# rfonod/geo-trax

Hardware: AMD Instinct MI355X
Metric: 4K frames/sec through detect+stabilize+track (higher is better)
Workload: dtype f32 (split-f16x3 MFMA)

## Files before the change

### geo-trax_amd/csrc/det_kernels.hip

```cpp
#include <hip/hip_runtime.h>

#include <mutex>
#include <hip/hip_fp16.h>

#include <cmath>

#include "det_kernels.hpp"

namespace gtx {

typedef _Float16 half8 __attribute__((ext_vector_type(8)));
typedef _Float16 half4 __attribute__((ext_vector_type(4)));

namespace {
inline double py_round(double v) { return std::nearbyint(v); }
}

Letterbox letterbox_geometry(int src_h, int src_w, int imgsz, bool rect, int stride) {
  Letterbox lb{};
  lb.src_h = src_h;
  lb.src_w = src_w;
  const double r = std::min((double)imgsz / src_h, (double)imgsz / src_w);
  lb.new_w = (int)py_round(src_w * r);
  lb.new_h = (int)py_round(src_h * r);
// ... 749 lines not shown

template <typename T> __device__ __forceinline__ float ldf(const T* p) { return (float)*p; }

__device__ __forceinline__ int find_level(const HeadParams& hp, int a) {
  int l = 0;
#pragma unroll
  for (int i = 1; i < kMaxLevels; ++i)
    if (i < hp.n_levels && a >= hp.lv[i].anchor_begin) l = i;
  return l;
}

template <typename T> __device__ __forceinline__ void load8(const T* p, float (&v)[8]);
template <> __device__ __forceinline__ void load8<_Float16>(const _Float16* p, float (&v)[8]) {
  const half8 h = *reinterpret_cast<const half8*>(p);
#pragma unroll
  for (int i = 0; i < 8; ++i) v[i] = (float)h[i];
}
template <> __device__ __forceinline__ void load8<float>(const float* p, float (&v)[8]) {
  const float4 a = reinterpret_cast<const float4*>(p)[0], b = reinterpret_cast<const float4*>(p)[1];
  v[0] = a.x; v[1] = a.y; v[2] = a.z; v[3] = a.w; v[4] = b.x; v[5] = b.y; v[6] = b.z; v[7] = b.w;
}

template <typename T>
__global__ __launch_bounds__(256) void head_candidates_kernel(const HeadParams hp, const NmsBuffers nb) {
  const int sub = threadIdx.x & 15;
  const int a = blockIdx.x * 16 + (threadIdx.x >> 4);
  const int n = blockIdx.y;
  const bool valid = a < hp.n_anchors;
  const int l = find_level(hp, valid ? a : 0);
  const HeadLevel& L = hp.lv[l];
  const int la = (valid ? a : 0) - L.anchor_begin;
  const T* fc = static_cast<const T*>(L.feat) + ((size_t)n * L.h * L.w + la) * L.cstride + L.cb;
  const int chunks = L.cc >> 3;
  float best = -1.f;
  int best_c = 0;
  for (int c0 = 0; c0 < hp.nc; c0 += 4) {
    float acc[4] = {0.f, 0.f, 0.f, 0.f};
    for (int ch = sub; ch < chunks; ch += 16) {
      float f[8];
      load8<T>(fc + ch * 8, f);
#pragma unroll
      for (int j = 0; j < 4; ++j) {
        if (c0 + j < hp.nc) {
          float w[8];
          load8<float>(L.wc + (size_t)(c0 + j) * L.cc + ch * 8, w);
#pragma unroll
          for (int e = 0; e < 8; ++e) acc[j] = fmaf(f[e], w[e], acc[j]);
// ... 92 lines not shown
}

template <typename T>
__global__ __launch_bounds__(256) void head_raw_kernel(const HeadParams hp, float* __restrict__ out, int logits) {
  const int n = blockIdx.y;
  const int lane = threadIdx.x & 63;
  const int a = (blockIdx.x * blockDim.x + threadIdx.x) >> 6;
  if (a >= hp.n_anchors) return;
  const int l = find_level(hp, a);
  const HeadLevel& L = hp.lv[l];
  const int la = a - L.anchor_begin;
  const T* f = static_cast<const T*>(L.feat) + ((size_t)n * L.h * L.w + la) * L.cstride;
  const float4 b = anchor_box<T>(L, f, la, lane);
  float* o = out + ((size_t)n * hp.n_anchors + a) * (4 + hp.nc);
  if (lane == 0) { o[0] = b.x; o[1] = b.y; o[2] = b.z; o[3] = b.w; }
  const T* fc = f + L.cb;
  for (int c = lane; c < hp.nc; c += 64) {
    float acc = L.bc[c];
    for (int k = 0; k < L.cc; ++k) acc = fmaf(ldf(fc + k), L.wc[c * L.cc + k], acc);
    o[4 + c] = logits ? acc : 1.f / (1.f + expf(-acc));
  }
}

void launch_head_candidates(int dtype, const HeadParams& hp, int n, const NmsBuffers& nb, hipStream_t s) {
  launch_head_gate(dtype, hp, n, nb, s);
  launch_head_boxes(dtype, hp, n, nb, s);
}

void launch_head_gate(int dtype, const HeadParams& hp, int n, const NmsBuffers& nb, hipStream_t s) {
  GTX_HIP(hipMemsetAsync(nb.count, 0, sizeof(int) * n, s));
  if (nb.lvl_count) GTX_HIP(hipMemsetAsync(nb.lvl_count, 0, sizeof(int) * n * kMaxLevels, s));
  dim3 grid(cdiv(hp.n_anchors, 16), n), block(256);
  if (dtype == DT_F16) hipLaunchKernelGGL(head_candidates_kernel<_Float16>, grid, block, 0, s, hp, nb);
  else hipLaunchKernelGGL(head_candidates_kernel<float>, grid, block, 0, s, hp, nb);
  GTX_HIP(hipGetLastError());
}

void launch_head_boxes(int dtype, const HeadParams& hp, int n, const NmsBuffers& nb, hipStream_t s) {
  dim3 grid2(64, n), block(256);
  const size_t lds = (size_t)hp.n_levels * hp.lv[0].cb * 64 * sizeof(float);
  GTX_CHECK(hp.n_levels <= kMaxLevels && hp.lv[0].cb <= 128, "head: %d levels of %d box channels", hp.n_levels, hp.lv[0].cb);
  static std::once_flag once;
  std::call_once(once, [] {
    GTX_HIP(hipFuncSetAttribute(reinterpret_cast<const void*>(head_boxes_kernel<_Float16>), hipFuncAttributeMaxDynamicSharedMemorySize, kMaxLevels * 128 * 64 * 4));
    GTX_HIP(hipFuncSetAttribute(reinterpret_cast<const void*>(head_boxes_kernel<float>), hipFuncAttributeMaxDynamicSharedMemorySize, kMaxLevels * 128 * 64 * 4));
  });
  if (dtype == DT_F16) hipLaunchKernelGGL(head_boxes_kernel<_Float16>, grid2, block, lds, s, hp, nb);
  else hipLaunchKernelGGL(head_boxes_kernel<float>, grid2, block, lds, s, hp, nb);
  GTX_HIP(hipGetLastError());
}

void launch_head_raw(int dtype, const HeadParams& hp, int n, float* out, bool logits, hipStream_t s) {
  dim3 grid(cdiv(hp.n_anchors * 64, 256), n), block(256);
  if (dtype == DT_F16) hipLaunchKernelGGL(head_raw_kernel<_Float16>, grid, block, 0, s, hp, out, logits ? 1 : 0);
  else hipLaunchKernelGGL(head_raw_kernel<float>, grid, block, 0, s, hp, out, logits ? 1 : 0);
  GTX_HIP(hipGetLastError());
}
// ... 163 lines not shown
    if (nb.out_anchor) nb.out_anchor[(size_t)n * nb.max_det + slot] = nb.s_anchor[(size_t)n * nb.nms_cap + i];
  }
}


__device__ __forceinline__ bool iou_gt(const float4& a, float area_a, const float4& b, float thr) {
  const float iw = fminf(a.z, b.z) - fmaxf(a.x, b.x);
  const float ih = fminf(a.w, b.w) - fmaxf(a.y, b.y);
  if (!(iw > 0.f && ih > 0.f)) return false;
  const float area_b = (b.z - b.x) * (b.w - b.y);
  const float inter = iw * ih;
  return inter / (area_a + area_b - inter) > thr;
}

__global__ __launch_bounds__(1024) void nms_small_kernel(const NmsBuffers nb, float thr, float cls_offset, float gain, float padx,
                                                         float pady, float fw, float fh) {
  __shared__ unsigned long long s_key[kSmallNms];
  __shared__ float4 s_box[kSmallNms];
  __shared__ float4 s_kbox[kSmallKeep];
  __shared__ int s_nkeep, s_done;
  const int n = blockIdx.x;
  const int tid = threadIdx.x, lane = tid & 63;
  const int wave = __builtin_amdgcn_readfirstlane(tid >> 6), nwaves = blockDim.x >> 6;
  const int cnt = min(nb.count[n], nb.cap);
  if (cnt > kSmallNms || nb.max_det > kSmallKeep) {
    if (tid == 0) nb.out_n[n] = 0;
    return;
  }
  if (tid == 0) { nb.sorted_n[n] = 0; s_nkeep = 0; s_done = 0; }
  const size_t base = (size_t)n * nb.cap;
  int P = 64;
  while (P < cnt) P <<= 1;
  for (int i = tid; i < P; i += blockDim.x) {
    unsigned long long k = 0ull;
    if (i < cnt) {
      const unsigned sb = __float_as_uint(nb.cand_score[base + i]);
      k = ((unsigned long long)sb << 32) | ((unsigned long long)(0x7FFFFu - (unsigned)nb.cand_anchor[base + i]) << 12) | (unsigned)i;
    }
    s_key[i] = k;
  }
  __syncthreads();
  for (int k = 2; k <= P; k <<= 1)
    for (int j = k >> 1; j > 0; j >>= 1) {
      for (int t = tid; t < P / 2; t += blockDim.x) {
        const int lo = ((t / j) * 2 * j) + (t % j), hi = lo + j;
        const bool desc = ((lo & k) == 0);
// ... 143 lines not shown
```

### geo-trax_amd/csrc/det_kernels.hpp

```cpp
#pragma once
#include <vector>

#include "common.hpp"
#include "conv_igemm.hpp"

namespace gtx {

struct Letterbox {
  int src_h, src_w;
  int net_h, net_w;
  int new_h, new_w;
  int top, left;
  double gain;
};
Letterbox letterbox_geometry(int src_h, int src_w, int imgsz, bool rect, int stride);

void launch_preprocess(int dtype, const uint8_t* frames, int n, const Letterbox& lb, void* img,
                       uint8_t* gray, int gh, int gw, hipStream_t s);

void launch_stem(int dtype, const void* img, int n, int h, int w, const float* w27, const float* bias,
                 const void* wpk_f16, int c0, void* out, int ho, int wo, hipStream_t s, float acc_scale = 1.f);
std::vector<uint16_t> pack_stem_weights_f16(const float* w27, int c0);
std::vector<uint16_t> pack_stem_weights_split(const float* w27, int c0, float* acc_scale);

// ... 24 lines not shown
};

struct NmsBuffers {
  int cap;
  int* count;
  float* cand_score;
  int* cand_anchor;
  int* cand_cls;
  float* cand_box;
  int nms_cap;
  int* sorted_n;
  float* s_box;
  float* s_score;
  int* s_cls;
  int* s_anchor;
  unsigned long long* mask;
  int max_det;
  int* out_n;
  float* out_rows;
  int* out_anchor;
  int* lvl_count;
  int* lvl_list;
  int lvl_cap;
};

struct FeatLevels {
  const void* feat[kMaxLevels];
  int h[kMaxLevels], w[kMaxLevels], cstride[kMaxLevels], coff[kMaxLevels], c[kMaxLevels];
  int anchor_begin[kMaxLevels];
  int n_levels;
  int dim;
};
void launch_obj_feats(int dtype, const FeatLevels& fl, int n, const NmsBuffers& nb, float* out, hipStream_t s);

void launch_head_candidates(int dtype, const HeadParams& hp, int n, const NmsBuffers& nb, hipStream_t s);
void launch_head_gate(int dtype, const HeadParams& hp, int n, const NmsBuffers& nb, hipStream_t s);
void launch_head_boxes(int dtype, const HeadParams& hp, int n, const NmsBuffers& nb, hipStream_t s);

struct SparseBoxLevel {
  const void* in;
  int H, W, cstride, coff, cin;
  const void* w1; const float* b1; float sc1;
  const void* w2; const float* b2; float sc2;
  int anchor_begin;
  const float* wb; const float* bb; float stride;
};
struct SparseBox {
  SparseBoxLevel lv[kMaxLevels];
  int n_levels;
  int cap;
  int* sat_flag;
};
void launch_head_sparse_box(const SparseBox& sb, int n, const NmsBuffers& nb, hipStream_t s);
void launch_head_raw(int dtype, const HeadParams& hp, int n, float* out, bool logits, hipStream_t s);
void launch_nms(const NmsBuffers& nb, int n, float iou_thr, bool agnostic, int max_nms,
                const Letterbox& lb, hipStream_t s, int which = 0);
bool nms_small_covers(int candidates, int max_det);

}
// ... 1 lines not shown
```

### geo-trax_amd/csrc/detector.cpp

```cpp
#include "detector.hpp"
#include "split_format.hpp"

#include <algorithm>
#include <array>
#include <cmath>
#include <deque>
#include <functional>
#include <mutex>

namespace gtx {

Detector::Detector(gtx_ctx* ctx, const gtx_det_config& cfg) : ctx_(ctx), cfg_(cfg) {
  GTX_CHECK(cfg.imgsz > 0 && cfg.imgsz % 32 == 0, "imgsz must be a positive multiple of 32 (got %d)", cfg.imgsz);
  GTX_CHECK(cfg.max_det > 0 && cfg.nc > 0 && cfg.nc <= 128, "max_det must be positive and nc in [1, 128] (got %d, %d)", cfg.max_det, cfg.nc);
  GTX_CHECK(cfg.frame_h > 0 && cfg.frame_w > 0, "frame size must be given");
  if (cfg_.max_batch < 1) cfg_.max_batch = 1;
  dtype_ = cfg.half ? DT_F16 : DT_F32;
  conv_dtype_ = (!cfg.half && cfg.fp32_split) ? DT_F32S : dtype_;
  es_ = dtype_size(dtype_);
  lb_ = letterbox_geometry(cfg.frame_h, cfg.frame_w, cfg.imgsz, cfg.rect != 0, 32);
  GTX_CHECK(lb_.net_h % 32 == 0 && lb_.net_w % 32 == 0, "network input %dx%d is not stride aligned", lb_.net_h, lb_.net_w);
  GTX_HIP(hipSetDevice(ctx->device));
  for (auto& e : ev_) GTX_HIP(hipEventCreateWithFlags(&e, wait_event_flags(true)));
  for (auto& e : ev_up_) GTX_HIP(hipEventCreate(&e));
}

Detector::~Detector() {
  if (h_out_n_) (void)hipHostFree(h_out_n_);
  if (h_sat_) (void)hipHostFree(h_sat_);
  if (h_out_rows_) (void)hipHostFree(h_out_rows_);
  if (h_feats_) (void)hipHostFree(h_feats_);
  if (h_count_) (void)hipHostFree(h_count_);
  for (auto& e : ev_)
    if (e) (void)hipEventDestroy(e);
  for (auto& e : ev_up_)
    if (e) (void)hipEventDestroy(e);
  for (auto& e : trace_ev_)
    if (e) (void)hipEventDestroy(e);
  if (graph_exec_) (void)hipGraphExecDestroy(graph_exec_);
}

void Detector::set_tensor(const std::string& name, const float* data, int ndim, const int64_t* shape) {
  GTX_CHECK(!finalized_, "set_tensor after finalize");
  HostTensor t;
  size_t n = 1;
  for (int i = 0; i < ndim; ++i) {
    t.shape.push_back(shape[i]);
    n *= (size_t)shape[i];
  }
  t.data.assign(data, data + n);
  tensors_[name] = std::move(t);
}

const HostTensor& Detector::tensor(const std::string& name) const {
  auto it = tensors_.find(name);
// ... 156 lines not shown
  int n = 0;
  while (has(pfx + ".m." + std::to_string(n) + ".cv1.conv.weight")) ++n;
  View cat = new_view(x.h, x.w, (2 + n) * c);
  View first = cat.slice(0, 2 * c);
  conv(pfx + ".cv1.conv", x, 1, true, &first, nullptr, up_src);
  for (int k = 0; k < n; ++k) {
    View tmp = new_view(x.h, x.w, c);
    const std::string m = pfx + ".m." + std::to_string(k);
    View src = cat.slice((1 + k) * c, c);
    View dst = cat.slice((2 + k) * c, c);
    conv(m + ".cv1.conv", src, 1, true, &tmp, nullptr);
    conv(m + ".cv2.conv", tmp, 1, true, &dst, shortcut ? &src : nullptr);
  }
  View out = conv(pfx + ".cv2.conv", cat, 1, true, out_slice, nullptr);
  layer_views_[pfx] = out;
  return out;
}

void Detector::build_graph() {
  const int H = lb_.net_h, W = lb_.net_w;
  img_ = new_view(H, W, 4);
  if (conv_dtype_ == DT_F32S) {
    sat_dev_ = (int*)alloc(sizeof(int));
    GTX_HIP(hipHostMalloc((void**)&h_sat_, sizeof(int)));
    *h_sat_ = 0;
  }

  const HostTensor& w0 = tensor("model.0.conv.weight");
  GTX_CHECK(w0.shape.size() == 4 && w0.shape[1] == 3 && w0.shape[2] == 3, "model.0 must be a 3x3 conv on 3 channels");
  const int c0 = (int)w0.shape[0];
  View a0 = new_view(H / 2, W / 2, c0);
  {
    std::vector<float> w27((size_t)27 * c0);
    for (int o = 0; o < c0; ++o)
      for (int i = 0; i < 3; ++i)
        for (int y = 0; y < 3; ++y)
          for (int x = 0; x < 3; ++x)
            w27[(size_t)((y * 3 + x) * 3 + i) * c0 + o] = w0.data[(((size_t)o * 3 + i) * 3 + y) * 3 + x];
    float* dw = (float*)alloc(w27.size() * sizeof(float));
    GTX_HIP(hipMemcpy(dw, w27.data(), w27.size() * sizeof(float), hipMemcpyHostToDevice));
    std::vector<float> b(c0, 0.f);
    if (has("model.0.conv.bias")) b = tensor("model.0.conv.bias").data;
    float* db = (float*)alloc((size_t)(c0 + 31) / 32 * 32 * sizeof(float));
    GTX_HIP(hipMemcpy(db, b.data(), c0 * sizeof(float), hipMemcpyHostToDevice));
    Op op;
    op.kind = Op::STEM;
    op.name = "model.0.conv";
    op.family = dtype_ == DT_F16 ? "stem_mfma_kernel" : (conv_dtype_ == DT_F32S ? "stem_split_kernel" : "stem_kernel");
// ... 533 lines not shown
    pad_skip_rows_ = 0;
    for (Op& op : ops_)
      for (int i = 0; i < kMaxGroup; ++i) op.ty_first[i] = op.ty_count[i] = 0;
    return;
  }
  pad_skip_on_ = true;
}

void Detector::finalize() {
  GTX_CHECK(!finalized_, "finalize called twice");
  GTX_HIP(hipSetDevice(ctx_->device));
  build_graph();
  fuse_front();
  fuse_stem();
  release_hidden_layers();
  const int N = cfg_.max_batch;
  gray_h_ = cfg_.frame_h / 2;
  gray_w_ = cfg_.frame_w / 2;
  gray_.alloc((size_t)kGrayRing * N * gray_h_ * gray_w_);
  nms_ = NmsBuffers{};
  nms_.cap = head_.n_anchors;
  nms_.nms_cap = 30016;
  nms_.max_det = cfg_.max_det;
  nms_.count = (int*)alloc(sizeof(int) * N);
  nms_.cand_score = (float*)alloc(sizeof(float) * N * nms_.cap);
  nms_.cand_anchor = (int*)alloc(sizeof(int) * N * nms_.cap);
  nms_.cand_cls = (int*)alloc(sizeof(int) * N * nms_.cap);
  nms_.cand_box = (float*)alloc(sizeof(float) * 4 * N * nms_.cap);
  nms_.sorted_n = (int*)alloc(sizeof(int) * N);
  nms_.s_box = (float*)alloc(sizeof(float) * 4 * N * nms_.nms_cap);
  nms_.s_score = (float*)alloc(sizeof(float) * N * nms_.nms_cap);
  nms_.s_cls = (int*)alloc(sizeof(int) * N * nms_.nms_cap);
  nms_.mask = (unsigned long long*)alloc(sizeof(unsigned long long) * N * (size_t)nms_.nms_cap * (nms_.nms_cap / 64));
  nms_.out_n = (int*)alloc(sizeof(int) * N);
  nms_.out_rows = (float*)alloc(sizeof(float) * 6 * N * cfg_.max_det);
  nms_.s_anchor = nms_.out_anchor = nullptr;
  if (cfg_.obj_feats) {
    nms_.s_anchor = (int*)alloc(sizeof(int) * N * nms_.nms_cap);
    nms_.out_anchor = (int*)alloc(sizeof(int) * N * cfg_.max_det);
    d_feats_ = (float*)alloc(sizeof(float) * N * cfg_.max_det * feat_levels_.dim);
    GTX_HIP(hipHostMalloc((void**)&h_feats_, sizeof(float) * N * cfg_.max_det * feat_levels_.dim));
  }
  if (sparse_on_) {
    sparse_.cap = kSparseCap;
    sparse_.sat_flag = sat_dev_;
    nms_.lvl_cap = kSparseCap;
    nms_.lvl_count = (int*)alloc(sizeof(int) * N * kMaxLevels);
    nms_.lvl_list = (int*)alloc(sizeof(int) * N * kMaxLevels * kSparseCap);
  }
  GTX_HIP(hipHostMalloc((void**)&h_count_, sizeof(int) * N));
  GTX_HIP(hipHostMalloc((void**)&h_out_n_, sizeof(int) * N));
  GTX_HIP(hipHostMalloc((void**)&h_out_rows_, sizeof(float) * 6 * N * cfg_.max_det));
  if (conv_dtype_ != DT_F32S) tensors_.clear();
  if (env_flag("GTX_PAD_SKIP", true)) {
    plan_pad_skip();
    prime_pad_skip();
  }
  set_batch(1);
  GTX_HIP(hipStreamSynchronize(ctx_->stream));
  finalized_ = true;
}

void Detector::run_op(const Op& op, int nb, hipStream_t s) {
  switch (op.kind) {
    case Op::CONV:
      conv_launch(op.grp, op.cfg, s);
      break;
    case Op::STEM:
      launch_stem(dtype_ == DT_F32 ? conv_dtype_ : dtype_, op.in.ptr, nb, op.in.h, op.in.w, op.w27, op.bias, op.wpk, op.out.c, op.out.ptr, op.out.h,
                  op.out.w, s, op.stem_scale);
      break;
    case Op::POOL: launch_sppf_pool(conv_dtype_ == DT_F32S ? DT_F32S : dtype_, op.out.ptr, nb, op.in.h, op.in.w, op.in.c, s); break;
    case Op::UPSAMPLE:
      launch_upsample2x(dtype_, op.in.ptr, nb, op.in.h, op.in.w, op.in.c, op.in.cstride, op.in.coff, op.out.ptr,
                        op.out.cstride, op.out.coff, s);
// ... 51 lines not shown
  for (size_t i = 0; i < ops_.size() && i < trace_n_.size(); ++i) {
    if (trace_n_[i] == 0) continue;
    auto it = idx.find(ops_[i].family);
    size_t k;
    if (it == idx.end()) {
      k = names.size();
      idx[ops_[i].family] = k;
      names.push_back(ops_[i].family);
      launches.push_back(0); ms.push_back(0.f); flops.push_back(0.0); bytes.push_back(0.0);
    } else {
      k = it->second;
    }
    launches[k] += trace_n_[i];
    ms[k] += (float)trace_ms_[i];
    flops[k] += trace_flops_[i];
    bytes[k] += trace_bytes_[i];
  }
  trace_ms_.assign(ops_.size(), 0.0);
  trace_n_.assign(ops_.size(), 0);
  trace_flops_.assign(ops_.size(), 0.0);
  trace_bytes_.assign(ops_.size(), 0.0);
}

void Detector::run_post(int nb, hipStream_t s) {
  if (sparse_on_) {
    launch_head_gate(dtype_, head_, nb, nms_, s);
    launch_head_sparse_box(sparse_, nb, nms_, s);
    dense_head_valid_ = false;
  } else {
    launch_head_candidates(dtype_, head_, nb, nms_, s);
  }
  GTX_HIP(hipMemcpyAsync(h_count_, nms_.count, sizeof(int) * nb, hipMemcpyDeviceToHost, s));
  launch_nms(nms_, nb, cfg_.iou, cfg_.agnostic_nms != 0, 30000, lb_, s, 1);
  GTX_HIP(hipMemcpyAsync(h_out_n_, nms_.out_n, sizeof(int) * nb, hipMemcpyDeviceToHost, s));
  GTX_HIP(hipMemcpyAsync(h_out_rows_, nms_.out_rows, sizeof(float) * 6 * nb * cfg_.max_det, hipMemcpyDeviceToHost, s));
  if (sat_dev_) GTX_HIP(hipMemcpyAsync(h_sat_, sat_dev_, sizeof(int), hipMemcpyDeviceToHost, s));
  if (cfg_.obj_feats) {
    launch_obj_feats(conv_dtype_, feat_levels_, nb, nms_, d_feats_, s);
    GTX_HIP(hipMemcpyAsync(h_feats_, d_feats_, sizeof(float) * nb * cfg_.max_det * feat_levels_.dim, hipMemcpyDeviceToHost, s));
  }
}

void Detector::run_dense_box(hipStream_t s) {
  if (!sparse_on_ || dense_head_valid_) return;
  GTX_CHECK(cur_nb_ > 0, "no forward pass has run yet");
  for (Op o : dense_box_ops_) {
    for (int i = 0; i < o.grp.count; ++i) o.grp.p[i].N = cur_nb_;
    conv_group_finalize(o.grp, o.cfg);
    run_op(o, cur_nb_, s);
  }
  dense_head_valid_ = true;
}

void Detector::features(int b, float* out, int cap, int* n, int* dim) const {
  if (exact_) return exact_->features(b, out, cap, n, dim);
  GTX_CHECK(cfg_.obj_feats && h_feats_, "features: the detector was created without gtx_det_config.obj_feats");
  GTX_CHECK(b >= 0 && b < cfg_.max_batch, "features: image %d of %d", b, cfg_.max_batch);
  const int cnt = std::min(b < (int)c_feat_n_.size() ? c_feat_n_[b] : 0, cap);
  if (n) *n = cnt;
// ... 76 lines not shown
      GTX_HIP(hipEventElapsedTime(&t, trace_ev_[i], trace_ev_[i + 1]));
      trace_ms_[i] += t;
      trace_n_[i] += 1;
      trace_flops_[i] += ops_[i].flops;
      trace_bytes_[i] += ops_[i].bytes;
    }
    flight_traced_ = false;
  }
  {
    bool over = false, big = false;
    for (int b = 0; b < flight_nb_; ++b) {
      over = over || (sparse_on_ && h_count_[b] > kSparseCap);
      big = big || !nms_small_covers(std::min(h_count_[b], nms_.cap), nms_.max_det);
    }
    if (over || big) {
      hipStream_t s = ctx_->stream;
      NmsBuffers dense = nms_;
      if (over) {
        run_dense_box(s);
        launch_head_boxes(dtype_, head_, flight_nb_, dense, s);
        ++sparse_overflows_;
      }
      launch_nms(dense, flight_nb_, cfg_.iou, cfg_.agnostic_nms != 0, 30000, lb_, s, over ? 0 : 2);
      GTX_HIP(hipMemcpyAsync(h_out_n_, nms_.out_n, sizeof(int) * flight_nb_, hipMemcpyDeviceToHost, s));
      GTX_HIP(hipMemcpyAsync(h_out_rows_, nms_.out_rows, sizeof(float) * 6 * flight_nb_ * cfg_.max_det, hipMemcpyDeviceToHost, s));
      if (cfg_.obj_feats) {
        launch_obj_feats(conv_dtype_, feat_levels_, flight_nb_, nms_, d_feats_, s);
        GTX_HIP(hipMemcpyAsync(h_feats_, d_feats_, sizeof(float) * flight_nb_ * cfg_.max_det * feat_levels_.dim, hipMemcpyDeviceToHost, s));
      }
      GTX_HIP(hipEventRecord(ev_[3], s));
      GTX_HIP(hipStreamSynchronize(s));
    }
  }
  const int nb = flight_nb_;
  if (cfg_.obj_feats) {
    c_feat_n_.assign(cfg_.max_batch, 0);
    c_feats_.resize((size_t)cfg_.max_batch * cfg_.max_det * feat_levels_.dim);
    for (int b = 0; b < nb; ++b) {
      c_feat_n_[b] = h_out_n_[b];
      const size_t o = (size_t)b * cfg_.max_det * feat_levels_.dim;
      memcpy(c_feats_.data() + o, h_feats_ + o, sizeof(float) * h_out_n_[b] * feat_levels_.dim);
    }
  }
  for (int b = 0; b < nb; ++b) {
    const int n = h_out_n_[b];
    n_out[b] = n;
    const float* rows = h_out_rows_ + (size_t)b * cfg_.max_det * 6;
    for (int i = 0; i < n; ++i) {
// ... 157 lines not shown
```

### geo-trax_amd/csrc/detector.hpp

```cpp
#pragma once
#include <map>
#include <memory>
#include <set>
#include <string>
#include <vector>

#include "../../include/gtx.h"
#include "common.hpp"
#include "conv_igemm.hpp"
#include "det_kernels.hpp"

struct gtx_ctx {
  int device = 0;
  hipStream_t stream = nullptr;
  hipDeviceProp_t prop{};
  ~gtx_ctx() {
    if (stream) (void)hipStreamDestroy(stream);
  }
};

namespace gtx {

struct HostTensor {
  std::vector<int64_t> shape;
// ... 139 lines not shown
  static constexpr int kGrayRing = 16;
  int gray_slot_ = 0, collected_gray_slot_ = 0;
  bool in_flight_ = false;
  int flight_nb_ = 0;

  HeadParams head_{};
  NmsBuffers nms_{};
  DevBuf raw_;
  int* sat_dev_ = nullptr;
  int* h_sat_ = nullptr;
  bool sat_seen_ = false;
  bool plain_out_ = false;
  std::vector<Op> unfused_;
  int* h_out_n_ = nullptr;
  FeatLevels feat_levels_{};
  static constexpr int kSparseCap = 8192;
  bool sparse_on_ = false;
  SparseBox sparse_{};
  Op head_ops_[kMaxLevels][3];
  std::string det_pfx_ = "model.22";
  std::vector<Op> dense_box_ops_;
  bool dense_head_valid_ = false;
  int* h_count_ = nullptr;
  int sparse_overflows_ = 0;
  void run_dense_box(hipStream_t s);
  bool pad_skip_on_ = false;
  int pad_skip_rows_ = 0, pad_skip_total_ = 0;
  void plan_pad_skip();
  void prime_pad_skip();
  float* d_feats_ = nullptr;
  float* h_feats_ = nullptr;
  std::vector<float> c_feats_;
  std::vector<int> c_feat_n_;
  float* h_out_rows_ = nullptr;
  hipEvent_t ev_[4]{};
  hipGraphExec_t graph_exec_ = nullptr;
  int graph_nb_ = 0;
  int trace_every_ = 0, trace_count_ = 0;
  bool flight_traced_ = false;
  std::vector<hipEvent_t> trace_ev_;
  std::vector<double> trace_ms_;
  std::vector<int> trace_n_;
  std::vector<double> trace_flops_, trace_bytes_;
  hipEvent_t ev_up_[2]{};
};

// ... 6 lines not shown
```

### geo-trax_amd/csrc/head_sparse.hip

```cpp
#include <hip/hip_runtime.h>
#include <hip/hip_fp16.h>

#include "det_kernels.hpp"

namespace gtx {

namespace {

typedef float floatx4 __attribute__((ext_vector_type(4)));
typedef _Float16 half8 __attribute__((ext_vector_type(8)));
typedef float float2v __attribute__((ext_vector_type(2)));
typedef _Float16 half2v __attribute__((ext_vector_type(2)));
#define GTXH_MFMA(a, b, c) __builtin_amdgcn_mfma_f32_16x16x32_f16(a, b, c, 0, 0, 0)

__device__ __forceinline__ float2v silu2(const float2v v) {
  const float2v t = v * -1.44269504088896341f;
  const float2v d = float2v{__builtin_amdgcn_exp2f(t.x), __builtin_amdgcn_exp2f(t.y)} + 1.f;
  return v * float2v{__builtin_amdgcn_rcpf(d.x), __builtin_amdgcn_rcpf(d.y)};
}
__device__ __forceinline__ void split2(const float2v v, unsigned& hi, unsigned& lo, bool& sat) {
  const float2v x = {__builtin_amdgcn_fmed3f(v.x, -65504.f, 65504.f), __builtin_amdgcn_fmed3f(v.y, -65504.f, 65504.f)};
  sat |= x.x != v.x || x.y != v.y;
  const half2v h = __builtin_convertvector(x, half2v);
  const half2v l = __builtin_convertvector(x - __builtin_convertvector(h, float2v), half2v);
  hi = __builtin_bit_cast(unsigned, h);
  lo = __builtin_bit_cast(unsigned, l);
}

constexpr int kRowBytes = 256;
constexpr int kCandPerWave = 4;
constexpr int kWaveLds = kCandPerWave * 9 * kRowBytes;

__device__ __forceinline__ const char* wrow(const void* w, int step , int row) {
  return static_cast<const char*>(w) + ((size_t)step * 64 + row) * 128;
}

__global__ __launch_bounds__(256) void head_sparse_box_kernel(const SparseBox sb, const NmsBuffers nb, int groups) {
  extern __shared__ __attribute__((aligned(16))) char smem[];
  const int n = blockIdx.y;
  const int l = blockIdx.x / groups, g = blockIdx.x - l * groups;
  const int lane = threadIdx.x & 63;
  const int wave = __builtin_amdgcn_readfirstlane(threadIdx.x >> 6);
  const int cnt = min(nb.lvl_count[n * kMaxLevels + l], nb.lvl_cap);
  const int first = (g * 4 + wave) * kCandPerWave;
  if (first >= cnt) return;
  const SparseBoxLevel& L = sb.lv[l];
  const int col = lane & 15, kg = lane >> 4;
  const int pos = min(col, 8);
  int ci[kCandPerWave], y1[kCandPerWave], x1[kCandPerWave];
  bool valid1[kCandPerWave];
#pragma unroll
  for (int c = 0; c < kCandPerWave; ++c) {
    const int k = min(first + c, cnt - 1);
    ci[c] = __builtin_amdgcn_readfirstlane(nb.lvl_list[((size_t)n * kMaxLevels + l) * nb.lvl_cap + k]);
    const int a = __builtin_amdgcn_readfirstlane(nb.cand_anchor[(size_t)n * nb.cap + ci[c]]);
    const int la = a - L.anchor_begin;
    const int ay = la / L.W, ax = la - ay * L.W;
    y1[c] = ay + pos / 3 - 1;
    x1[c] = ax + pos % 3 - 1;
    valid1[c] = y1[c] >= 0 && y1[c] < L.H && x1[c] >= 0 && x1[c] < L.W;
  }
  const float* __restrict__ in = static_cast<const float*>(L.in) + (size_t)n * L.H * L.W * L.cstride + L.coff + kg * 8;
  char* lds = smem + wave * kWaveLds;

  floatx4 acc[kCandPerWave][4];
  {
    const float inv_sc = __builtin_amdgcn_rcpf(L.sc1);
#pragma unroll
    for (int q = 0; q < 4; ++q) {
      const float4 b = *reinterpret_cast<const float4*>(L.b1 + 16 * q + 4 * kg);
#pragma unroll
      for (int c = 0; c < kCandPerWave; ++c) acc[c][q] = floatx4{b.x * inv_sc, b.y * inv_sc, b.z * inv_sc, b.w * inv_sc};
    }
  }
  const int nsteps = (L.cin / 32) * 9;
  half8 bh[3][kCandPerWave], bl[3][kCandPerWave], ah[3][4], al[3][4];
#define GTXH_LOAD1(STEP, R)                                                                     \
  {                                                                                             \
    const int ch__ = (STEP) / 9, tap__ = (STEP) - ch__ * 9;                                     \
    _Pragma("unroll") for (int c = 0; c < kCandPerWave; ++c) {                                  \
      const int y__ = y1[c] + tap__ / 3 - 1, x__ = x1[c] + tap__ % 3 - 1;                       \
      uint4 h__ = make_uint4(0, 0, 0, 0), l__ = make_uint4(0, 0, 0, 0);                         \
      if (y__ >= 0 && y__ < L.H && x__ >= 0 && x__ < L.W) {                                     \
        const uint4* s__ = reinterpret_cast<const uint4*>(in + ((size_t)y__ * L.W + x__) * L.cstride + ch__ * 32); \
        h__ = s__[0];                                                                           \
        l__ = s__[1];                                                                           \
      }                                                                                         \
      bh[R][c] = __builtin_bit_cast(half8, h__);                                                \
      bl[R][c] = __builtin_bit_cast(half8, l__);                                                \
    }                                                                                           \
    _Pragma("unroll") for (int q = 0; q < 4; ++q) {                                             \
      const int row__ = 16 * q + col;                                                           \
      const char* w__ = wrow(L.w1, STEP, row__);                                                \
      ah[R][q] = *reinterpret_cast<const half8*>(w__ + ((kg ^ ((row__ >> 1) & 7)) << 4));       \
      al[R][q] = *reinterpret_cast<const half8*>(w__ + (((4 + kg) ^ ((row__ >> 1) & 7)) << 4)); \
    }                                                                                           \
  }
#define GTXH_STEP1(S, R)                                                                        \
  {                                                                                             \
    if ((S) + 2 < nsteps) GTXH_LOAD1((S) + 2, ((R) + 2) % 3)                                    \
    _Pragma("unroll") for (int c = 0; c < kCandPerWave; ++c)                                    \
      _Pragma("unroll") for (int q = 0; q < 4; ++q) {                                           \
        acc[c][q] = GTXH_MFMA(al[R][q], bh[R][c], acc[c][q]);                                   \
        acc[c][q] = GTXH_MFMA(ah[R][q], bl[R][c], acc[c][q]);                                   \
        acc[c][q] = GTXH_MFMA(ah[R][q], bh[R][c], acc[c][q]);                                   \
      }                                                                                         \
  }
  GTXH_LOAD1(0, 0)
  GTXH_LOAD1(1, 1)
  for (int s = 0; s < nsteps; s += 3) {
    GTXH_STEP1(s, 0)
    GTXH_STEP1(s + 1, 1)
    GTXH_STEP1(s + 2, 2)
  }
#undef GTXH_STEP1
#undef GTXH_LOAD1
  bool sat = false;
#pragma unroll
  for (int c = 0; c < kCandPerWave; ++c)
#pragma unroll
    for (int q = 0; q < 4; ++q) {
      float2v v[2];
#pragma unroll
      for (int e = 0; e < 2; ++e) {
        v[e] = silu2(float2v{acc[c][q][2 * e], acc[c][q][2 * e + 1]} * L.sc1);
        if (!valid1[c]) v[e] = float2v{0.f, 0.f};
      }
      uint2 hi, lo;
      bool s1 = false;
      split2(v[0], hi.x, lo.x, s1);
      split2(v[1], hi.y, lo.y, s1);
      sat |= s1 && col < 9;
      const auto sx = __builtin_amdgcn_permlane16_swap(hi.x, lo.x, false, false);
      const auto sy = __builtin_amdgcn_permlane16_swap(hi.y, lo.y, false, false);
      if (col < 9) *reinterpret_cast<uint4*>(lds + (c * 9 + col) * kRowBytes + 64 * q + 16 * kg) = make_uint4(sx[0], sy[0], sx[1], sy[1]);
    }

  floatx4 acc2[4];
  {
    const float inv_sc = __builtin_amdgcn_rcpf(L.sc2);
#pragma unroll
    for (int q = 0; q < 4; ++q) {
      const float4 b = *reinterpret_cast<const float4*>(L.b2 + 16 * q + 4 * kg);
      acc2[q] = floatx4{b.x * inv_sc, b.y * inv_sc, b.z * inv_sc, b.w * inv_sc};
    }
  }
  const char* mine = lds + (col & 3) * 9 * kRowBytes;
  half8 wh[3][4], wl[3][4];
#define GTXH_LOAD2(STEP, R)                                                                     \
  _Pragma("unroll") for (int q = 0; q < 4; ++q) {                                               \
    const int row__ = 16 * q + col;                                                             \
    const char* w__ = wrow(L.w2, STEP, row__);                                                  \
    wh[R][q] = *reinterpret_cast<const half8*>(w__ + ((kg ^ ((row__ >> 1) & 7)) << 4));         \
    wl[R][q] = *reinterpret_cast<const half8*>(w__ + (((4 + kg) ^ ((row__ >> 1) & 7)) << 4));   \
  }
#define GTXH_STEP2(S, R)                                                                        \
  {                                                                                             \
    if ((S) + 2 < 18) GTXH_LOAD2((S) + 2, ((R) + 2) % 3)                                        \
    const int ch__ = (S) / 9, tap__ = (S) - ch__ * 9;                                           \
    const char* r__ = mine + tap__ * kRowBytes + (4 * ch__ + kg) * 32;    \
    const half8 xh__ = *reinterpret_cast<const half8*>(r__), xl__ = *reinterpret_cast<const half8*>(r__ + 16); \
    _Pragma("unroll") for (int q = 0; q < 4; ++q) {                                             \
      acc2[q] = GTXH_MFMA(wl[R][q], xh__, acc2[q]);                                             \
      acc2[q] = GTXH_MFMA(wh[R][q], xl__, acc2[q]);                                             \
      acc2[q] = GTXH_MFMA(wh[R][q], xh__, acc2[q]);                                             \
    }                                                                                           \
  }
  GTXH_LOAD2(0, 0)
  GTXH_LOAD2(1, 1)
#pragma unroll 1
  for (int s = 0; s < 18; s += 3) {
    GTXH_STEP2(s, 0)
    GTXH_STEP2(s + 1, 1)
    GTXH_STEP2(s + 2, 2)
  }
#undef GTXH_STEP2
#undef GTXH_LOAD2
  float* fl = reinterpret_cast<float*>(lds);
  if (col < kCandPerWave) {
#pragma unroll
    for (int q = 0; q < 4; ++q) {
      const float2v v0 = silu2(float2v{acc2[q][0], acc2[q][1]} * L.sc2), v1 = silu2(float2v{acc2[q][2], acc2[q][3]} * L.sc2);
      *reinterpret_cast<float4*>(fl + col * 64 + 16 * q + 4 * kg) = make_float4(v0.x, v0.y, v1.x, v1.y);
    }
  }
#pragma unroll 1
  for (int c = 0; c < kCandPerWave; ++c) {
    if (first + c >= cnt) break;
    float a = L.bb[lane];
    const float* wr = L.wb + lane;
#pragma unroll 8
    for (int k = 0; k < 64; ++k) a = fmaf(fl[c * 64 + k], wr[(size_t)k * 64], a);
    const int anchor = __builtin_amdgcn_readfirstlane(nb.cand_anchor[(size_t)n * nb.cap + ci[c]]);
    const int la = anchor - L.anchor_begin;
    float m = a;
#pragma unroll
    for (int o = 8; o >= 1; o >>= 1) m = fmaxf(m, __shfl_xor(m, o, 64));
    const float e = expf(a - m);
    float se = e, sw = e * (float)(lane & 15);
#pragma unroll
    for (int o = 8; o >= 1; o >>= 1) {
      se += __shfl_xor(se, o, 64);
      sw += __shfl_xor(sw, o, 64);
    }
    const float d = sw / se;
    const float d0 = __shfl(d, 0, 64), d1 = __shfl(d, 16, 64), d2 = __shfl(d, 32, 64), d3 = __shfl(d, 48, 64);
    const float ax = (float)(la % L.W) + 0.5f, ay = (float)(la / L.W) + 0.5f;
    const float bx1 = ax - d0, by1 = ay - d1, bx2 = ax + d2, by2 = ay + d3;
    const float4 b = make_float4((bx1 + bx2) * 0.5f * L.stride, (by1 + by2) * 0.5f * L.stride, (bx2 - bx1) * L.stride, (by2 - by1) * L.stride);
    if (lane == 0) {
      const float hw = b.z / 2.f, hh = b.w / 2.f;
      reinterpret_cast<float4*>(nb.cand_box)[(size_t)n * nb.cap + ci[c]] = make_float4(b.x - hw, b.y - hh, b.x + hw, b.y + hh);
    }
  }
  if (sb.sat_flag && __builtin_amdgcn_ballot_w64(sat) != 0 && lane == 0) atomicOr(sb.sat_flag, 1);
}

}

void launch_head_sparse_box(const SparseBox& sb, int n, const NmsBuffers& nb, hipStream_t s) {
  GTX_CHECK(sb.cap > 0 && nb.lvl_count != nullptr && nb.lvl_list != nullptr && nb.lvl_cap == sb.cap, "sparse box branch: no buffers");
  const int groups = (nb.lvl_cap + 4 * kCandPerWave - 1) / (4 * kCandPerWave);
  hipLaunchKernelGGL(head_sparse_box_kernel, dim3(sb.n_levels * groups, n), dim3(256), 4 * kWaveLds, s, sb, nb, groups);
  GTX_HIP(hipGetLastError());
}

}
```

Before: 1117.

## Double-buffer result buffers, fuse zeroing into gate kernel, persistent sparse-box kernel

Counters and result buffers now live in two contiguous device sets that alternate each frame. The next set is zeroed inside the gate kernel instead of by separate memsets, and a single D2H copy brings back counts, out_n, sat flag and rows together instead of four copies. The sparse box kernel becomes a persistent grid (two blocks per CU) that walks levels and images with a work counter, one candidate per wave by default, and pads its LDS row stride. This trades launch, memset and copy overhead and idle blocks for more complex buffer bookkeeping and less MFMA reuse per wave.

```diff
diff --git a/geo-trax_amd/csrc/det_kernels.hip b/geo-trax_amd/csrc/det_kernels.hip
--- a/geo-trax_amd/csrc/det_kernels.hip
+++ b/geo-trax_amd/csrc/det_kernels.hip
@@ -795,7 +795,10 @@
 }
 
 template <typename T>
-__global__ __launch_bounds__(256) void head_candidates_kernel(const HeadParams hp, const NmsBuffers nb) {
+__global__ __launch_bounds__(256) void head_candidates_kernel(const HeadParams hp, const NmsBuffers nb, int* __restrict__ zero_next,
+                                                               int zero_ints) {
+  if (blockIdx.x == 0 && blockIdx.y == 0)
+    for (int i = threadIdx.x; i < zero_ints; i += blockDim.x) zero_next[i] = 0;
   const int sub = threadIdx.x & 15;
   const int a = blockIdx.x * 16 + (threadIdx.x >> 4);
   const int n = blockIdx.y;
@@ -934,17 +937,20 @@
   }
 }
 
-void launch_head_candidates(int dtype, const HeadParams& hp, int n, const NmsBuffers& nb, hipStream_t s) {
-  launch_head_gate(dtype, hp, n, nb, s);
+void launch_head_candidates(int dtype, const HeadParams& hp, int n, const NmsBuffers& nb, hipStream_t s, int* zero_next, int zero_ints) {
+  launch_head_gate(dtype, hp, n, nb, s, zero_next, zero_ints);
   launch_head_boxes(dtype, hp, n, nb, s);
 }
 
-void launch_head_gate(int dtype, const HeadParams& hp, int n, const NmsBuffers& nb, hipStream_t s) {
-  GTX_HIP(hipMemsetAsync(nb.count, 0, sizeof(int) * n, s));
-  if (nb.lvl_count) GTX_HIP(hipMemsetAsync(nb.lvl_count, 0, sizeof(int) * n * kMaxLevels, s));
+void launch_head_gate(int dtype, const HeadParams& hp, int n, const NmsBuffers& nb, hipStream_t s, int* zero_next, int zero_ints) {
+  if (!zero_next) {
+    GTX_HIP(hipMemsetAsync(nb.count, 0, sizeof(int) * n, s));
+    if (nb.lvl_count) GTX_HIP(hipMemsetAsync(nb.lvl_count, 0, sizeof(int) * n * kMaxLevels, s));
+    zero_ints = 0;
+  }
   dim3 grid(cdiv(hp.n_anchors, 16), n), block(256);
-  if (dtype == DT_F16) hipLaunchKernelGGL(head_candidates_kernel<_Float16>, grid, block, 0, s, hp, nb);
-  else hipLaunchKernelGGL(head_candidates_kernel<float>, grid, block, 0, s, hp, nb);
+  if (dtype == DT_F16) hipLaunchKernelGGL(head_candidates_kernel<_Float16>, grid, block, 0, s, hp, nb, zero_next, zero_ints);
+  else hipLaunchKernelGGL(head_candidates_kernel<float>, grid, block, 0, s, hp, nb, zero_next, zero_ints);
   GTX_HIP(hipGetLastError());
 }
 
@@ -1154,6 +1160,7 @@
   const int n = blockIdx.x;
   const int tid = threadIdx.x, lane = tid & 63;
   const int wave = __builtin_amdgcn_readfirstlane(tid >> 6), nwaves = blockDim.x >> 6;
+  if (n == 0 && tid == 0 && nb.sat_dst) *nb.sat_dst = nb.sat_src ? *nb.sat_src : 0;
   const int cnt = min(nb.count[n], nb.cap);
   if (cnt > kSmallNms || nb.max_det > kSmallKeep) {
     if (tid == 0) nb.out_n[n] = 0;
diff --git a/geo-trax_amd/csrc/det_kernels.hpp b/geo-trax_amd/csrc/det_kernels.hpp
--- a/geo-trax_amd/csrc/det_kernels.hpp
+++ b/geo-trax_amd/csrc/det_kernels.hpp
@@ -70,6 +70,8 @@
   int* lvl_count;
   int* lvl_list;
   int lvl_cap;
+  const int* sat_src;
+  int* sat_dst;
 };
 
 struct FeatLevels {
@@ -81,8 +83,10 @@
 };
 void launch_obj_feats(int dtype, const FeatLevels& fl, int n, const NmsBuffers& nb, float* out, hipStream_t s);
 
-void launch_head_candidates(int dtype, const HeadParams& hp, int n, const NmsBuffers& nb, hipStream_t s);
-void launch_head_gate(int dtype, const HeadParams& hp, int n, const NmsBuffers& nb, hipStream_t s);
+void launch_head_candidates(int dtype, const HeadParams& hp, int n, const NmsBuffers& nb, hipStream_t s, int* zero_next = nullptr,
+                            int zero_ints = 0);
+void launch_head_gate(int dtype, const HeadParams& hp, int n, const NmsBuffers& nb, hipStream_t s, int* zero_next = nullptr,
+                      int zero_ints = 0);
 void launch_head_boxes(int dtype, const HeadParams& hp, int n, const NmsBuffers& nb, hipStream_t s);
 
 struct SparseBoxLevel {
diff --git a/geo-trax_amd/csrc/detector.cpp b/geo-trax_amd/csrc/detector.cpp
--- a/geo-trax_amd/csrc/detector.cpp
+++ b/geo-trax_amd/csrc/detector.cpp
@@ -26,11 +26,8 @@
 }
 
 Detector::~Detector() {
-  if (h_out_n_) (void)hipHostFree(h_out_n_);
-  if (h_sat_) (void)hipHostFree(h_sat_);
-  if (h_out_rows_) (void)hipHostFree(h_out_rows_);
+  if (h_res_) (void)hipHostFree(h_res_);
   if (h_feats_) (void)hipHostFree(h_feats_);
-  if (h_count_) (void)hipHostFree(h_count_);
   for (auto& e : ev_)
     if (e) (void)hipEventDestroy(e);
   for (auto& e : ev_up_)
@@ -233,8 +230,6 @@
   img_ = new_view(H, W, 4);
   if (conv_dtype_ == DT_F32S) {
     sat_dev_ = (int*)alloc(sizeof(int));
-    GTX_HIP(hipHostMalloc((void**)&h_sat_, sizeof(int)));
-    *h_sat_ = 0;
   }
 
   const HostTensor& w0 = tensor("model.0.conv.weight");
@@ -814,7 +809,6 @@
   nms_.cap = head_.n_anchors;
   nms_.nms_cap = 30016;
   nms_.max_det = cfg_.max_det;
-  nms_.count = (int*)alloc(sizeof(int) * N);
   nms_.cand_score = (float*)alloc(sizeof(float) * N * nms_.cap);
   nms_.cand_anchor = (int*)alloc(sizeof(int) * N * nms_.cap);
   nms_.cand_cls = (int*)alloc(sizeof(int) * N * nms_.cap);
@@ -824,8 +818,6 @@
   nms_.s_score = (float*)alloc(sizeof(float) * N * nms_.nms_cap);
   nms_.s_cls = (int*)alloc(sizeof(int) * N * nms_.nms_cap);
   nms_.mask = (unsigned long long*)alloc(sizeof(unsigned long long) * N * (size_t)nms_.nms_cap * (nms_.nms_cap / 64));
-  nms_.out_n = (int*)alloc(sizeof(int) * N);
-  nms_.out_rows = (float*)alloc(sizeof(float) * 6 * N * cfg_.max_det);
   nms_.s_anchor = nms_.out_anchor = nullptr;
   if (cfg_.obj_feats) {
     nms_.s_anchor = (int*)alloc(sizeof(int) * N * nms_.nms_cap);
@@ -837,12 +829,21 @@
     sparse_.cap = kSparseCap;
     sparse_.sat_flag = sat_dev_;
     nms_.lvl_cap = kSparseCap;
-    nms_.lvl_count = (int*)alloc(sizeof(int) * N * kMaxLevels);
     nms_.lvl_list = (int*)alloc(sizeof(int) * N * kMaxLevels * kSparseCap);
   }
-  GTX_HIP(hipHostMalloc((void**)&h_count_, sizeof(int) * N));
-  GTX_HIP(hipHostMalloc((void**)&h_out_n_, sizeof(int) * N));
-  GTX_HIP(hipHostMalloc((void**)&h_out_rows_, sizeof(float) * 6 * N * cfg_.max_det));
+  res_count_off_ = N * kMaxLevels;
+  res_zero_ints_ = N * (kMaxLevels + 1);
+  res_rows_off_ = (res_count_off_ + 2 * N + 1 + 3) & ~3;
+  const size_t res_ints = (size_t)res_rows_off_ + (size_t)6 * N * cfg_.max_det;
+  for (auto& r : res_) r = (int*)alloc(sizeof(int) * res_ints);
+  GTX_HIP(hipHostMalloc((void**)&h_res_, sizeof(int) * (res_ints - res_count_off_)));
+  memset(h_res_, 0, sizeof(int) * (res_ints - res_count_off_));
+  h_count_ = h_res_;
+  h_out_n_ = h_res_ + N;
+  h_sat_ = h_res_ + 2 * N;
+  h_out_rows_ = reinterpret_cast<float*>(h_res_ + (res_rows_off_ - res_count_off_));
+  nms_.sat_src = sat_dev_;
+  use_result_set(0);
   if (conv_dtype_ != DT_F32S) tensors_.clear();
   if (env_flag("GTX_PAD_SKIP", true)) {
     plan_pad_skip();
@@ -940,19 +941,34 @@
   trace_bytes_.assign(ops_.size(), 0.0);
 }
 
+void Detector::use_result_set(int set) {
+  const int N = cfg_.max_batch;
+  res_set_ = set;
+  int* r = res_[set];
+  nms_.lvl_count = sparse_on_ ? r : nullptr;
+  nms_.count = r + res_count_off_;
+  nms_.out_n = r + res_count_off_ + N;
+  nms_.sat_dst = r + res_count_off_ + 2 * N;
+  nms_.out_rows = reinterpret_cast<float*>(r + res_rows_off_);
+}
+
+void Detector::copy_results(int nb, hipStream_t s) {
+  const size_t ints = (size_t)(res_rows_off_ - res_count_off_) + (size_t)6 * nb * cfg_.max_det;
+  GTX_HIP(hipMemcpyAsync(h_res_, res_[res_set_] + res_count_off_, sizeof(int) * ints, hipMemcpyDeviceToHost, s));
+}
+
 void Detector::run_post(int nb, hipStream_t s) {
+  use_result_set(res_set_ ^ 1);
+  int* zero_next = res_[res_set_ ^ 1];
   if (sparse_on_) {
-    launch_head_gate(dtype_, head_, nb, nms_, s);
+    launch_head_gate(dtype_, head_, nb, nms_, s, zero_next, res_zero_ints_);
     launch_head_sparse_box(sparse_, nb, nms_, s);
     dense_head_valid_ = false;
   } else {
-    launch_head_candidates(dtype_, head_, nb, nms_, s);
-  }
-  GTX_HIP(hipMemcpyAsync(h_count_, nms_.count, sizeof(int) * nb, hipMemcpyDeviceToHost, s));
+    launch_head_candidates(dtype_, head_, nb, nms_, s, zero_next, res_zero_ints_);
+  }
   launch_nms(nms_, nb, cfg_.iou, cfg_.agnostic_nms != 0, 30000, lb_, s, 1);
-  GTX_HIP(hipMemcpyAsync(h_out_n_, nms_.out_n, sizeof(int) * nb, hipMemcpyDeviceToHost, s));
-  GTX_HIP(hipMemcpyAsync(h_out_rows_, nms_.out_rows, sizeof(float) * 6 * nb * cfg_.max_det, hipMemcpyDeviceToHost, s));
-  if (sat_dev_) GTX_HIP(hipMemcpyAsync(h_sat_, sat_dev_, sizeof(int), hipMemcpyDeviceToHost, s));
+  copy_results(nb, s);
   if (cfg_.obj_feats) {
     launch_obj_feats(conv_dtype_, feat_levels_, nb, nms_, d_feats_, s);
     GTX_HIP(hipMemcpyAsync(h_feats_, d_feats_, sizeof(float) * nb * cfg_.max_det * feat_levels_.dim, hipMemcpyDeviceToHost, s));
@@ -1075,8 +1091,7 @@
         ++sparse_overflows_;
       }
       launch_nms(dense, flight_nb_, cfg_.iou, cfg_.agnostic_nms != 0, 30000, lb_, s, over ? 0 : 2);
-      GTX_HIP(hipMemcpyAsync(h_out_n_, nms_.out_n, sizeof(int) * flight_nb_, hipMemcpyDeviceToHost, s));
-      GTX_HIP(hipMemcpyAsync(h_out_rows_, nms_.out_rows, sizeof(float) * 6 * flight_nb_ * cfg_.max_det, hipMemcpyDeviceToHost, s));
+      copy_results(flight_nb_, s);
       if (cfg_.obj_feats) {
         launch_obj_feats(conv_dtype_, feat_levels_, flight_nb_, nms_, d_feats_, s);
         GTX_HIP(hipMemcpyAsync(h_feats_, d_feats_, sizeof(float) * flight_nb_ * cfg_.max_det * feat_levels_.dim, hipMemcpyDeviceToHost, s));
diff --git a/geo-trax_amd/csrc/detector.hpp b/geo-trax_amd/csrc/detector.hpp
--- a/geo-trax_amd/csrc/detector.hpp
+++ b/geo-trax_amd/csrc/detector.hpp
@@ -185,6 +185,12 @@
   std::vector<Op> dense_box_ops_;
   bool dense_head_valid_ = false;
   int* h_count_ = nullptr;
+  int* res_[2] = {nullptr, nullptr};
+  int res_set_ = 0;
+  int* h_res_ = nullptr;
+  int res_count_off_ = 0, res_rows_off_ = 0, res_zero_ints_ = 0;
+  void use_result_set(int set);
+  void copy_results(int nb, hipStream_t s);
   int sparse_overflows_ = 0;
   void run_dense_box(hipStream_t s);
   bool pad_skip_on_ = false;
diff --git a/geo-trax_amd/csrc/head_sparse.hip b/geo-trax_amd/csrc/head_sparse.hip
--- a/geo-trax_amd/csrc/head_sparse.hip
+++ b/geo-trax_amd/csrc/head_sparse.hip
@@ -1,5 +1,8 @@
 #include <hip/hip_runtime.h>
 #include <hip/hip_fp16.h>
+
+#include <algorithm>
+#include <cstdlib>
 
 #include "det_kernels.hpp"
 
@@ -28,29 +31,23 @@
 }
 
 constexpr int kRowBytes = 256;
-constexpr int kCandPerWave = 4;
-constexpr int kWaveLds = kCandPerWave * 9 * kRowBytes;
+constexpr int kRowStride = kRowBytes + 16;
+constexpr int kWavesPerGroup = 4;
 
 __device__ __forceinline__ const char* wrow(const void* w, int step , int row) {
   return static_cast<const char*>(w) + ((size_t)step * 64 + row) * 128;
 }
 
-__global__ __launch_bounds__(256) void head_sparse_box_kernel(const SparseBox sb, const NmsBuffers nb, int groups) {
-  extern __shared__ __attribute__((aligned(16))) char smem[];
-  const int n = blockIdx.y;
-  const int l = blockIdx.x / groups, g = blockIdx.x - l * groups;
-  const int lane = threadIdx.x & 63;
-  const int wave = __builtin_amdgcn_readfirstlane(threadIdx.x >> 6);
-  const int cnt = min(nb.lvl_count[n * kMaxLevels + l], nb.lvl_cap);
-  const int first = (g * 4 + wave) * kCandPerWave;
-  if (first >= cnt) return;
+template <int kCand>
+__device__ __forceinline__ void sparse_box_group(const SparseBox& sb, const NmsBuffers& nb, int n, int l, int first, int cnt,
+                                                 char* lds, int lane, bool& sat) {
   const SparseBoxLevel& L = sb.lv[l];
   const int col = lane & 15, kg = lane >> 4;
   const int pos = min(col, 8);
-  int ci[kCandPerWave], y1[kCandPerWave], x1[kCandPerWave];
-  bool valid1[kCandPerWave];
-#pragma unroll
-  for (int c = 0; c < kCandPerWave; ++c) {
+  int ci[kCand], y1[kCand], x1[kCand];
+  bool valid1[kCand];
+#pragma unroll
+  for (int c = 0; c < kCand; ++c) {
     const int k = min(first + c, cnt - 1);
     ci[c] = __builtin_amdgcn_readfirstlane(nb.lvl_list[((size_t)n * kMaxLevels + l) * nb.lvl_cap + k]);
     const int a = __builtin_amdgcn_readfirstlane(nb.cand_anchor[(size_t)n * nb.cap + ci[c]]);
@@ -61,24 +58,23 @@
     valid1[c] = y1[c] >= 0 && y1[c] < L.H && x1[c] >= 0 && x1[c] < L.W;
   }
   const float* __restrict__ in = static_cast<const float*>(L.in) + (size_t)n * L.H * L.W * L.cstride + L.coff + kg * 8;
-  char* lds = smem + wave * kWaveLds;
-
-  floatx4 acc[kCandPerWave][4];
+
+  floatx4 acc[kCand][4];
   {
     const float inv_sc = __builtin_amdgcn_rcpf(L.sc1);
 #pragma unroll
     for (int q = 0; q < 4; ++q) {
       const float4 b = *reinterpret_cast<const float4*>(L.b1 + 16 * q + 4 * kg);
 #pragma unroll
-      for (int c = 0; c < kCandPerWave; ++c) acc[c][q] = floatx4{b.x * inv_sc, b.y * inv_sc, b.z * inv_sc, b.w * inv_sc};
+      for (int c = 0; c < kCand; ++c) acc[c][q] = floatx4{b.x * inv_sc, b.y * inv_sc, b.z * inv_sc, b.w * inv_sc};
     }
   }
   const int nsteps = (L.cin / 32) * 9;
-  half8 bh[3][kCandPerWave], bl[3][kCandPerWave], ah[3][4], al[3][4];
+  half8 bh[3][kCand], bl[3][kCand], ah[3][4], al[3][4];
 #define GTXH_LOAD1(STEP, R)                                                                     \
   {                                                                                             \
     const int ch__ = (STEP) / 9, tap__ = (STEP) - ch__ * 9;                                     \
-    _Pragma("unroll") for (int c = 0; c < kCandPerWave; ++c) {                                  \
+    _Pragma("unroll") for (int c = 0; c < kCand; ++c) {                                  \
       const int y__ = y1[c] + tap__ / 3 - 1, x__ = x1[c] + tap__ % 3 - 1;                       \
       uint4 h__ = make_uint4(0, 0, 0, 0), l__ = make_uint4(0, 0, 0, 0);                         \
       if (y__ >= 0 && y__ < L.H && x__ >= 0 && x__ < L.W) {                                     \
@@ -99,7 +95,7 @@
 #define GTXH_STEP1(S, R)                                                                        \
   {                                                                                             \
     if ((S) + 2 < nsteps) GTXH_LOAD1((S) + 2, ((R) + 2) % 3)                                    \
-    _Pragma("unroll") for (int c = 0; c < kCandPerWave; ++c)                                    \
+    _Pragma("unroll") for (int c = 0; c < kCand; ++c)                                    \
       _Pragma("unroll") for (int q = 0; q < 4; ++q) {                                           \
         acc[c][q] = GTXH_MFMA(al[R][q], bh[R][c], acc[c][q]);                                   \
         acc[c][q] = GTXH_MFMA(ah[R][q], bl[R][c], acc[c][q]);                                   \
@@ -115,9 +111,8 @@
   }
 #undef GTXH_STEP1
 #undef GTXH_LOAD1
-  bool sat = false;
-#pragma unroll
-  for (int c = 0; c < kCandPerWave; ++c)
+#pragma unroll
+  for (int c = 0; c < kCand; ++c)
 #pragma unroll
     for (int q = 0; q < 4; ++q) {
       float2v v[2];
@@ -133,7 +128,7 @@
       sat |= s1 && col < 9;
       const auto sx = __builtin_amdgcn_permlane16_swap(hi.x, lo.x, false, false);
       const auto sy = __builtin_amdgcn_permlane16_swap(hi.y, lo.y, false, false);
-      if (col < 9) *reinterpret_cast<uint4*>(lds + (c * 9 + col) * kRowBytes + 64 * q + 16 * kg) = make_uint4(sx[0], sy[0], sx[1], sy[1]);
+      if (col < 9) *reinterpret_cast<uint4*>(lds + (c * 9 + col) * kRowStride + 64 * q + 16 * kg) = make_uint4(sx[0], sy[0], sx[1], sy[1]);
     }
 
   floatx4 acc2[4];
@@ -145,7 +140,7 @@
       acc2[q] = floatx4{b.x * inv_sc, b.y * inv_sc, b.z * inv_sc, b.w * inv_sc};
     }
   }
-  const char* mine = lds + (col & 3) * 9 * kRowBytes;
+  const char* mine = lds + (col % kCand) * 9 * kRowStride;
   half8 wh[3][4], wl[3][4];
 #define GTXH_LOAD2(STEP, R)                                                                     \
   _Pragma("unroll") for (int q = 0; q < 4; ++q) {                                               \
@@ -158,7 +153,7 @@
   {                                                                                             \
     if ((S) + 2 < 18) GTXH_LOAD2((S) + 2, ((R) + 2) % 3)                                        \
     const int ch__ = (S) / 9, tap__ = (S) - ch__ * 9;                                           \
-    const char* r__ = mine + tap__ * kRowBytes + (4 * ch__ + kg) * 32;    \
+    const char* r__ = mine + tap__ * kRowStride + (4 * ch__ + kg) * 32;    \
     const half8 xh__ = *reinterpret_cast<const half8*>(r__), xl__ = *reinterpret_cast<const half8*>(r__ + 16); \
     _Pragma("unroll") for (int q = 0; q < 4; ++q) {                                             \
       acc2[q] = GTXH_MFMA(wl[R][q], xh__, acc2[q]);                                             \
@@ -177,7 +172,7 @@
 #undef GTXH_STEP2
 #undef GTXH_LOAD2
   float* fl = reinterpret_cast<float*>(lds);
-  if (col < kCandPerWave) {
+  if (col < kCand) {
 #pragma unroll
     for (int q = 0; q < 4; ++q) {
       const float2v v0 = silu2(float2v{acc2[q][0], acc2[q][1]} * L.sc2), v1 = silu2(float2v{acc2[q][2], acc2[q][3]} * L.sc2);
@@ -185,7 +180,7 @@
     }
   }
 #pragma unroll 1
-  for (int c = 0; c < kCandPerWave; ++c) {
+  for (int c = 0; c < kCand; ++c) {
     if (first + c >= cnt) break;
     float a = L.bb[lane];
     const float* wr = L.wb + lane;
@@ -213,16 +208,52 @@
       reinterpret_cast<float4*>(nb.cand_box)[(size_t)n * nb.cap + ci[c]] = make_float4(b.x - hw, b.y - hh, b.x + hw, b.y + hh);
     }
   }
+}
+
+template <int kCand>
+__global__ __launch_bounds__(256) void head_sparse_box_kernel(const SparseBox sb, const NmsBuffers nb, int n_img) {
+  extern __shared__ __attribute__((aligned(16))) char smem[];
+  const int lane = threadIdx.x & 63;
+  const int wave = __builtin_amdgcn_readfirstlane(threadIdx.x >> 6);
+  const int nw = gridDim.x * kWavesPerGroup;
+  char* lds = smem + wave * (kCand * 9 * kRowStride);
+  bool sat = false;
+  int item = blockIdx.x * kWavesPerGroup + wave;
+  for (int l = sb.n_levels - 1; l >= 0; --l)
+    for (int n = 0; n < n_img; ++n) {
+      const int cnt = __builtin_amdgcn_readfirstlane(min(nb.lvl_count[n * kMaxLevels + l], nb.lvl_cap));
+      const int groups = (cnt + kCand - 1) / kCand;
+      for (; item < groups; item += nw) sparse_box_group<kCand>(sb, nb, n, l, item * kCand, cnt, lds, lane, sat);
+      item -= groups;
+    }
   if (sb.sat_flag && __builtin_amdgcn_ballot_w64(sat) != 0 && lane == 0) atomicOr(sb.sat_flag, 1);
+}
+
+template <int kCand>
+void launch_cand(const SparseBox& sb, int n, const NmsBuffers& nb, hipStream_t s) {
+  static const int groups = [] {
+    int dev = 0, cus = 0;
+    GTX_HIP(hipGetDevice(&dev));
+    GTX_HIP(hipDeviceGetAttribute(&cus, hipDeviceAttributeMultiprocessorCount, dev));
+    return 2 * std::max(cus, 1);
+  }();
+  hipLaunchKernelGGL(head_sparse_box_kernel<kCand>, dim3(groups), dim3(64 * kWavesPerGroup), kWavesPerGroup * kCand * 9 * kRowStride, s,
+                     sb, nb, n);
+  GTX_HIP(hipGetLastError());
 }
 
 }
 
 void launch_head_sparse_box(const SparseBox& sb, int n, const NmsBuffers& nb, hipStream_t s) {
   GTX_CHECK(sb.cap > 0 && nb.lvl_count != nullptr && nb.lvl_list != nullptr && nb.lvl_cap == sb.cap, "sparse box branch: no buffers");
-  const int groups = (nb.lvl_cap + 4 * kCandPerWave - 1) / (4 * kCandPerWave);
-  hipLaunchKernelGGL(head_sparse_box_kernel, dim3(sb.n_levels * groups, n), dim3(256), 4 * kWaveLds, s, sb, nb, groups);
-  GTX_HIP(hipGetLastError());
-}
-
-}
+  static const int cand = [] {
+    const char* e = getenv("GTX_SPARSE_CAND");
+    const int v = e ? atoi(e) : 1;
+    return v == 2 || v == 4 ? v : 1;
+  }();
+  if (cand == 1) launch_cand<1>(sb, n, nb, s);
+  else if (cand == 4) launch_cand<4>(sb, n, nb, s);
+  else launch_cand<2>(sb, n, nb, s);
+}
+
+}
```

After: 1119 (median of 6 runs). No clear change (+0.1%).
